# Kateridge/TransMF_AD

Hardware: AMD Instinct MI355X
Metric: volume-pairs/sec fwd+bwd(+Adam), 96^3 MRI+PET batch=8 per GPU (higher is better)
Workload: dtype f32

## Files before the change

### transmf_ad_amd/csrc/conv1_fused.hip

```cpp
#include <type_traits>
#include "conv1_z.h"

namespace {
using namespace c1z;

enum { MODE_STATS = 0, MODE_FWD = 1, MODE_REDUCE = 2, MODE_WGRAD = 3, MODE_RD = 4 };
#ifndef TMF_C1X_LAZY
#define TMF_C1X_LAZY 0x12
#endif

struct Args {
    const float* x;
    const float* w;
    const float* scale;
    const float* shift;
    const float* mean;
    const float* invstd;
    const float* coef;
    const void* dpool;
    void* pooled;
    float* zsel;
    unsigned char* parg;
    float* partial;
    float* partial2;
    int D, H, W, C;
    int tilesD, tilesH, tilesW, ntiles, tiles_per_block;
    float slope;
};

template <int MODE, bool BF16, bool P16 = false, bool SPLIT = false, bool ROUTE = false>
__global__ __launch_bounds__(256, (MODE == 3 && !SPLIT) || (MODE == 1 && SPLIT) ? 4 : 2) void conv1_fused_kernel(Args a) {
    static_assert(!(BF16 && SPLIT), "SPLIT is the fp32 mode's variant");
    static_assert(!ROUTE || (!BF16 && !P16 && (MODE == MODE_FWD || (MODE == MODE_RD && !SPLIT))),
                  "ROUTE: the fp32 forward (either form of z) and the one-pass backward, which evaluates no z and so has one form");
    constexpr bool NOZ = ROUTE && MODE == MODE_RD;
    constexpr bool B16L = BF16 || SPLIT;
    constexpr int NIMG = SPLIT ? 3 : 1;
    constexpr bool KEEP32 = SPLIT && (MODE == MODE_RD || MODE == MODE_WGRAD);
    __shared__ float halo[B16L ? NIMG * NHB_DW : NHALO];
    __shared__ float halo32[KEEP32 ? NHALO : 1];
    const unsigned hb_base = (unsigned)(size_t)(__attribute__((address_space(3))) const void*)halo;
    __shared__ float red[4 * 32 * 32];
    const int tid = threadIdx.x;
    const int lane = tid & 63;
    const int wave = __builtin_amdgcn_readfirstlane(tid >> 6);
    const int l31 = lane & 31, hsel = lane >> 5;
    const int n0 = blockIdx.y * 32;
    const int co = n0 + l31;
    const bool cv = co < a.C;
    const int OD = a.D / 2, OH = a.H / 2, OW = a.W / 2;

    float bw[B16L ? 1 : 14];
    tmf_bf16x8 bwb[NIMG][3];
    if constexpr (B16L) weights_b16<SPLIT>(a.w, a.C, co, cv, hsel, bwb);
    else if constexpr (!NOZ) weights_f32(a.w, a.C, co, cv, hsel, bw);
    float sc = 0.f, sh = 0.f, mu = 0.f, is = 0.f, c0 = 0.f, c1 = 0.f;
    if (MODE != MODE_STATS && cv) { sc = a.scale[co]; sh = a.shift[co]; }
    if ((MODE == MODE_REDUCE || MODE == MODE_WGRAD || MODE == MODE_RD) && cv) { mu = a.mean[co]; is = a.invstd[co]; }
    if (MODE == MODE_WGRAD && cv) { c0 = a.coef[co]; c1 = a.coef[a.C + co]; }

    float s1 = 0.f, s2 = 0.f;
    float dacc[MODE == MODE_RD ? 27 : 1];
#pragma unroll
    for (int t = 0; t < (MODE == MODE_RD ? 27 : 1); ++t) dacc[t] = 0.f;
    f32x16 accw;
#pragma unroll
    for (int r = 0; r < 16; ++r) accw[r] = 0.f;
    const int a_tap = tapoff(l31);
    const int wg_tap = l31 < 27 ? l31 : 0, wg_c = (wg_tap % 3) & 1;
    const unsigned wg_b = hb_base + 2u * (unsigned)((wg_tap / 9) * BPLANE + ((wg_tap / 3) % 3) * BROW + wg_tap % 3 + wg_c +
                                                    wg_c * BCOPY + 2 * hsel * BROW);

    const int tile_begin = blockIdx.x * a.tiles_per_block;
    int tile_end = tile_begin + a.tiles_per_block;
    if (tile_end > a.ntiles) tile_end = a.ntiles;

    constexpr int OOB = (int)0x80000000u;
    constexpr int HVN = (NHALO + 255) / 256;
    float hv[HVN];
    int hrel[HVN], hcrd[HVN], hdst[HVN];
#pragma unroll
    for (int q = 0; q < HVN; ++q) {
        const int e = tid + q * 256;
        const int hw = e % HW, hh = (e / HW) % HH, hd = e / (HW * HH);
        hrel[q] = e < NHALO ? ((hd * a.H + hh) * a.W + hw) * 4 : OOB;
        hcrd[q] = hd | hh << 8 | hw << 16;
        hdst[q] = hd * BPLANE + hh * BROW + hw;
    }
    if (B16L) {
        for (int e = tid; e < NIMG * NHB_DW; e += 256) halo[e] = 0.f;
        __syncthreads();
    }
    auto min_i = [](int x_, int y_) { return x_ < y_ ? x_ : y_; };
    struct Crd { int tw, th, td, b; long xoff; bool in_dh, full_dh; };
    const bool even_dims = (a.D % 2 == 0) && (a.H % 2 == 0) && (a.W % 2 == 0);
    auto row_setup = [&](Crd& c) {
        const int d0 = c.td * TD, h0 = c.th * TH;
        c.xoff = (long)c.b * a.D * a.H * a.W + ((long)((d0 - 1) * a.H + (h0 - 1)) * a.W + (c.tw * TW - 1));
        c.in_dh = d0 >= 1 && d0 + TD < a.D && h0 >= 1 && h0 + TH < a.H;
        c.full_dh = d0 + TD <= a.D && h0 + TH <= a.H && even_dims;
    };
    auto next_crd = [&](Crd c) {
        c.xoff += TW;
        if (++c.tw == a.tilesW) {
            c.tw = 0;
            if (++c.th == a.tilesH) {
                c.th = 0;
                if (++c.td == a.tilesD) { c.td = 0; ++c.b; }
            }
            row_setup(c);
        }
        return c;
    };
    auto fetch = [&](const Crd& c) {
        const int d0 = c.td * TD, h0 = c.th * TH, w0 = c.tw * TW;
        const float* org = a.x + c.xoff;
        const __amdgpu_buffer_rsrc_t xr = __builtin_amdgcn_make_buffer_rsrc(const_cast<float*>(org), 0, 0x7FFFFFFF, 0x00020000);
        if (c.in_dh && w0 >= 1 && w0 + TW < a.W) {
#pragma unroll
            for (int q = 0; q < HVN; ++q)
                hv[q] = __builtin_bit_cast(float, __builtin_amdgcn_raw_buffer_load_b32(xr, hrel[q], 0, 0));
        } else {
            const int lo = (d0 == 0 ? 1 : 0) | (h0 == 0 ? 1 : 0) << 8 | (w0 == 0 ? 1 : 0) << 16;
            const int hi = min_i(HD - 1, a.D - d0) | min_i(HH - 1, a.H - h0) << 8 | min_i(HW - 1, a.W - w0) << 16;
            const unsigned lo_bias = 0x808080u - (unsigned)lo, hi_bias = (unsigned)hi | 0x808080u;
#pragma unroll
            for (int q = 0; q < HVN; ++q) {
                const unsigned tt = (unsigned)hcrd[q] + lo_bias, uu = hi_bias - (unsigned)hcrd[q];
                const int off = (((tt & uu) | ~0x808080u) == 0xFFFFFFFFu) ? hrel[q] : OOB;
                hv[q] = __builtin_bit_cast(float, __builtin_amdgcn_raw_buffer_load_b32(xr, off, 0, 0));
            }
        }
    };
    constexpr int PSZ = P16 ? 2 : 4;
    const int pl_lane = cv ? (hsel * OW * a.C + co) * PSZ : OOB;
    Crd cur;
    {
        int t = tile_begin;
        cur.tw = t % a.tilesW; t /= a.tilesW;
        cur.th = t % a.tilesH; t /= a.tilesH;
        cur.td = t % a.tilesD;
        cur.b = t / a.tilesD;
        row_setup(cur);
    }
    if (tile_begin < tile_end) fetch(cur);
    for (int tile = tile_begin; tile < tile_end; ++tile) {
        const int b = cur.b;
        const int d0 = cur.td * TD, h0 = cur.th * TH, w0 = cur.tw * TW;
        const bool full = cur.full_dh && w0 + TW <= a.W;
        cur = next_crd(cur);
        if (tile > tile_begin) __syncthreads();
        constexpr bool REDST = SPLIT && ROUTE && MODE == MODE_FWD;
        int tid_b = tid;
        if (REDST) asm volatile("" : "+v"(tid_b));
#pragma unroll
        for (int q = 0; q < HVN; ++q) {
            const int e = tid + q * 256;
            if (REDST) {
                const int eb = tid_b + q * 256;
                hdst[q] = (eb / (HW * HH)) * BPLANE + ((eb / HW) % HH) * BROW + eb % HW;
            }
            if (SPLIT) {
                if (e < NHALO) {
                    store_halo_split(halo, hdst[q], hv[q]);
                    if (KEEP32) halo32[e] = hv[q];
                }
            } else if (BF16) {
                if (e < NHALO) store_halo_bf16(halo, hdst[q], hv[q]);
            } else {
                if (e < NHALO) halo[e] = hv[q];
            }
        }
        __syncthreads();
        if (tile + 1 < tile_end) fetch(cur);

        auto process = [&](auto full_c) {
        constexpr bool FULL = decltype(full_c)::value;
        f32x16 zt[NTI];
        constexpr bool LAZY = (BF16 && MODE == MODE_WGRAD) || (SPLIT && ((TMF_C1X_LAZY >> MODE) & 1));
        const int i = l31;
        const unsigned lane_b = lane_base(hb_base, i, hsel);
        auto conv_tiles = [&](f32x16* zp, int mt0, auto n_c) {
            constexpr int N = decltype(n_c)::value;
            if constexpr (B16L) conv_tiles_b16<SPLIT, N>(zp, lane_b, mt0, bwb);
            else conv_tiles_f32<N>(zp, halo, mt0, vox_off(i), hsel, bw);
        };
        if (!LAZY && !NOZ) conv_tiles(zt, wave * NTI, std::integral_constant<int, NTI>{});
#pragma unroll
        for (int ti = 0; ti < NTI; ++ti) {
            const int mt = wave * NTI + ti;
            const int org = tile_org(mt);
            if (LAZY) conv_tiles(&zt[ti], mt, std::integral_constant<int, 1>{});
            f32x16& z = zt[ti];
            const int bd = d0 + 2 * (mt >> 2), bh = h0 + 4 * ((mt >> 1) & 1) + 2 * hsel, bwid = w0 + 4 * (mt & 1);

            if (MODE == MODE_STATS) {
#pragma unroll
                for (int r = 0; r < 16; ++r) {
                    const int gd = bd + ((r >> 2) & 1), gh = bh + ((r >> 1) & 1), gw = bwid + 2 * ((r >> 3) & 1) + (r & 1);
                    if (FULL || (gd < a.D && gh < a.H && gw < a.W)) { s1 += z[r]; s2 += z[r] * z[r]; }
                }
                continue;
            }

            float K0 = 0.f, K1 = 0.f;
            if (MODE == MODE_WGRAD) {
                K1 = -sc * c1 * is;
                K0 = sc * (c1 * mu * is - c0);
            }
            const int od = (d0 >> 1) + (mt >> 2), ohb = (h0 >> 1) + 2 * ((mt >> 1) & 1), owb = (w0 >> 1) + 2 * (mt & 1);
            void* pbase = MODE == MODE_FWD ? a.pooled : const_cast<void*>(a.dpool);
            const __amdgpu_buffer_rsrc_t pr = __builtin_amdgcn_make_buffer_rsrc(
                reinterpret_cast<char*>(pbase) + (size_t)b * OD * OH * OW * a.C * PSZ, 0, OD * OH * OW * a.C * PSZ, 0x00020000);
            const int pv = (FULL || ohb + hsel < OH) ? pl_lane : OOB;
            const __amdgpu_buffer_rsrc_t zr = __builtin_amdgcn_make_buffer_rsrc(
                reinterpret_cast<char*>(a.zsel) + (ROUTE ? (size_t)b * OD * OH * OW * a.C * 4 : 0), 0, ROUTE ? OD * OH * OW * a.C * 4 : 0, 0x00020000);
            const __amdgpu_buffer_rsrc_t ar = __builtin_amdgcn_make_buffer_rsrc(
                a.parg + (ROUTE ? (size_t)b * OD * OH * OW * a.C : 0), 0, ROUTE ? OD * OH * OW * a.C : 0, 0x00020000);
#pragma unroll
            for (int q = 0; q < 2; ++q) {
                const int ow = owb + q;
                const bool win_u = FULL || (od < OD && ow < OW);
                const int psoff = ((od * OH + ohb) * OW + ow) * a.C * PSZ;
                if (NOZ) {
                    float g = 0.f, zs = 0.f;
                    int arg = 0;
                    if (win_u) {
                        g = __builtin_bit_cast(float, __builtin_amdgcn_raw_buffer_load_b32(pr, pv, psoff, 0));
                        zs = __builtin_bit_cast(float, __builtin_amdgcn_raw_buffer_load_b32(zr, pv, psoff, 0));
                        arg = __builtin_amdgcn_raw_buffer_load_b8(ar, (int)((unsigned)pv >> 2), psoff / PSZ, 0) & 7;
                    }
                    const float gl = g * (zs * sc + sh > 0.f ? 1.f : a.slope);
                    s1 += gl;
                    s2 += gl * ((zs - mu) * is);
                    const int vx = org + hsel * 2 * HW + ((arg >> 2) & 1) * HH * HW + ((arg >> 1) & 1) * HW + 2 * q + (arg & 1);
#pragma unroll
                    for (int t = 0; t < 27; ++t) dacc[t] = fmaf(halo[vx + tapoff(t)], gl, dacc[t]);
                    continue;
                }
                float y[8];
                window_y(z, q, sc, sh, y);
                const float ymax = window_max(y);
                const float lrm = ymax > 0.f ? 1.f : a.slope;
                if (MODE == MODE_FWD) {
                    const float best = ymax * lrm;
                    if ((TMF_C1X_ABL & 1) && best == 12345.678f) __builtin_amdgcn_raw_buffer_store_b32(__builtin_bit_cast(unsigned, best), pr, pv, psoff, 0);
                    if (win_u && !(TMF_C1X_ABL & 1)) {
                        if (P16) __builtin_amdgcn_raw_buffer_store_b16((unsigned short)(tmf_pack_bf16(best, 0.f) & 0xFFFFu), pr, pv, psoff, 0);
                        else __builtin_amdgcn_raw_buffer_store_b32(__builtin_bit_cast(unsigned, best), pr, pv, psoff, 0);
                        if (ROUTE) {
                            const float zs = window_zsel(y, ymax, z, q);
                            const int arg = window_arg(y, ymax);
                            __builtin_amdgcn_raw_buffer_store_b32(__builtin_bit_cast(unsigned, zs), zr, pv, psoff, 0);
                            __builtin_amdgcn_raw_buffer_store_b8((unsigned char)arg, ar, (int)((unsigned)pv >> 2), psoff / PSZ, 0);
                        }
                    }
                    continue;
                }
                float g = 0.f;
                if (win_u)
                    g = P16 ? __builtin_bit_cast(float, (unsigned int)__builtin_amdgcn_raw_buffer_load_b16(pr, pv, psoff, 0) << 16)
                            : __builtin_bit_cast(float, __builtin_amdgcn_raw_buffer_load_b32(pr, pv, psoff, 0));
                const float gl = g * lrm;
                if (MODE == MODE_REDUCE || MODE == MODE_RD) {
                    const float zs = window_zsel(y, ymax, z, q);
                    s1 += gl;
                    s2 += gl * ((zs - mu) * is);
                    if (MODE == MODE_RD) {
                        const int arg = window_arg(y, ymax);
                        if (BF16) {
                            const int hd = 2 * (mt >> 2) + ((arg >> 2) & 1), hh = 4 * ((mt >> 1) & 1) + 2 * hsel + ((arg >> 1) & 1);
                            const unsigned short* hb = reinterpret_cast<const unsigned short*>(halo) + hd * BPLANE + hh * BROW +
                                                       4 * (mt & 1) + 2 * q + (arg & 1);
#pragma unroll
                            for (int t = 0; t < 27; ++t) {
                                const float xv = __builtin_bit_cast(float, (unsigned int)hb[(t / 9) * BPLANE + ((t / 3) % 3) * BROW + t % 3] << 16);
                                dacc[t] = fmaf(xv, gl, dacc[t]);
                            }
                        } else {
                        const int vx = org + hsel * 2 * HW + ((arg >> 2) & 1) * HH * HW + ((arg >> 1) & 1) * HW + 2 * q + (arg & 1);
                        const float* h32 = KEEP32 ? halo32 : halo;
#pragma unroll
                        for (int t = 0; t < 27; ++t) dacc[t] = fmaf(h32[vx + tapoff(t)], gl, dacc[t]);
                        }
                    }
                } else {
                    const int arg = window_arg(y, ymax);
                    const float add = sc * gl;
#pragma unroll
                    for (int k = 0; k < 8; ++k) {
                        const int r = 8 * q + k;
                        const int gd = bd + ((r >> 2) & 1), gh = bh + ((r >> 1) & 1), gw = bwid + 2 * q + (r & 1);
                        const bool vv = FULL || (gd < a.D && gh < a.H && gw < a.W);
                        const float dzv = z[r] * K1 + K0 + (k == arg ? add : 0.f);
                        z[r] = (vv && cv) ? dzv : 0.f;
                    }
                }
            }
            if (MODE == MODE_WGRAD) {
                const int a_row = org + hsel * 2 * HW + a_tap;
                if (BF16) {
                    const unsigned wt = wg_b + 2u * (unsigned)((2 * (mt >> 2)) * BPLANE + 4 * ((mt >> 1) & 1) * BROW + 4 * (mt & 1));
#pragma unroll
                    for (int m = 0; m < 2; ++m) {
                        float bv[8];
                        unsigned ad[4];
#pragma unroll
                        for (int u = 0; u < 4; ++u)
                            ad[u] = *reinterpret_cast<const __attribute__((address_space(3))) unsigned*>(
                                (size_t)(wt + 2u * (unsigned)((u >> 1) * BPLANE + (u & 1) * BROW + 2 * m)));
#pragma unroll
                        for (int j = 0; j < 8; ++j) bv[j] = z[8 * m + j];
                        const tmf_u32x4 av = {ad[0], ad[1], ad[2], ad[3]};
                        accw = __builtin_amdgcn_mfma_f32_32x32x16_bf16(__builtin_bit_cast(tmf_bf16x8, av), pack8(bv), accw, 0, 0, 0);
                    }
                } else {
#pragma unroll
                    for (int r = 0; r < 16; ++r)
                        accw = __builtin_amdgcn_mfma_f32_32x32x2f32((KEEP32 ? halo32 : halo)[a_row + row_off(r)], z[r], accw, 0, 0, 0);
                }
            }
        }
        };
        if (full)
            process(std::true_type{});
        else
            process(std::false_type{});
    }

    if (MODE == MODE_STATS || MODE == MODE_REDUCE || MODE == MODE_RD) {
        s1 += __shfl_xor(s1, 32);
        s2 += __shfl_xor(s2, 32);
        __syncthreads();
        if (hsel == 0) { red[(wave * 32 + l31) * 2] = s1; red[(wave * 32 + l31) * 2 + 1] = s2; }
        __syncthreads();
        if (tid < 32 && n0 + tid < a.C) {
            float t1 = 0.f, t2 = 0.f;
#pragma unroll
            for (int m = 0; m < 4; ++m) { t1 += red[(m * 32 + tid) * 2]; t2 += red[(m * 32 + tid) * 2 + 1]; }
            a.partial[((size_t)blockIdx.x * 2 + 0) * a.C + n0 + tid] = t1;
            a.partial[((size_t)blockIdx.x * 2 + 1) * a.C + n0 + tid] = t2;
        }
    }
    if (MODE == MODE_RD) {
        __syncthreads();
#pragma unroll
        for (int t = 0; t < 27; ++t) {
            const float v = dacc[t] + __shfl_xor(dacc[t], 32);
            if (hsel == 0) red[(wave * 32 + t) * 32 + l31] = v;
        }
        __syncthreads();
        for (int e = tid; e < 27 * 32; e += 256) {
            const int tap = e >> 5, c = e & 31;
            if (n0 + c < a.C) {
                const float v = red[(0 * 32 + tap) * 32 + c] + red[(1 * 32 + tap) * 32 + c] +
                                red[(2 * 32 + tap) * 32 + c] + red[(3 * 32 + tap) * 32 + c];
                a.partial2[((size_t)blockIdx.x * 27 + tap) * a.C + n0 + c] = v;
            }
        }
    } else if (MODE == MODE_WGRAD) {
        __syncthreads();
#pragma unroll
        for (int r = 0; r < 16; ++r) {
            const int tap = (r & 3) + 8 * (r >> 2) + 4 * hsel;
            red[(wave * 32 + tap) * 32 + l31] = accw[r];
        }
        __syncthreads();
        for (int e = tid; e < 27 * 32; e += 256) {
            const int tap = e >> 5, c = e & 31;
            if (n0 + c < a.C) {
                const float v = red[(0 * 32 + tap) * 32 + c] + red[(1 * 32 + tap) * 32 + c] +
                                red[(2 * 32 + tap) * 32 + c] + red[(3 * 32 + tap) * 32 + c];
                a.partial[((size_t)blockIdx.x * 27 + tap) * a.C + n0 + c] = v;
            }
        }
    }
}

struct Plan { int tilesD, tilesH, tilesW, ntiles, nby, tpb, nblk; };
Plan make_plan(int B, int D, int H, int W, int C, int target_blocks) {
    Plan p;
    p.tilesD = tmf_cdiv(D, TD); p.tilesH = tmf_cdiv(H, TH); p.tilesW = tmf_cdiv(W, TW);
    p.ntiles = B * p.tilesD * p.tilesH * p.tilesW;
    p.nby = tmf_cdiv(C, 32);
    int want = target_blocks / p.nby;
    if (want < 1) want = 1;
    if (want > p.ntiles) want = p.ntiles;
    p.tpb = tmf_cdiv(p.ntiles, want);
    p.nblk = tmf_cdiv(p.ntiles, p.tpb);
    return p;
}
#define SLAB_BLOCKS tmf_opt(TMF_OPT_C1_BLOCKS)

int check(const char* fn, int B, int D, int H, int W, int C) { return check_shape(fn, B, D, H, W, C); }

Args base_args(const float* x, const float* w, int D, int H, int W, int C, const Plan& p, float slope) {
    Args a = {};
    a.x = x; a.w = w; a.D = D; a.H = H; a.W = W; a.C = C;
    a.tilesD = p.tilesD; a.tilesH = p.tilesH; a.tilesW = p.tilesW; a.ntiles = p.ntiles; a.tiles_per_block = p.tpb;
    a.slope = slope;
    return a;
}

int c1_split_mode() { return tmf_opt(TMF_OPT_C1_SPLIT); }

}

extern "C" int tmf_c1_blocks(int B, int D, int H, int W, int C) {
    if (B <= 0 || D <= 0 || H <= 0 || W <= 0 || C <= 0) return 0;
    return make_plan(B, D, H, W, C, SLAB_BLOCKS).nblk;
}

static int c1_stats(bool bf16, const float* x, const float* w, float* stat_partial,
                    int B, int D, int H, int W, int C, void* stream) {
    TMF_REQUIRE_PTR(x); TMF_REQUIRE_PTR(w); TMF_REQUIRE_PTR(stat_partial);
    int rc = check("tmf_c1_stats", B, D, H, W, C);
    if (rc) return rc;
    const Plan p = make_plan(B, D, H, W, C, SLAB_BLOCKS);
    Args a = base_args(x, w, D, H, W, C, p, 0.f);
    a.partial = stat_partial;
    if (bf16) hipLaunchKernelGGL((conv1_fused_kernel<MODE_STATS, true>), dim3(p.nblk, p.nby), dim3(256), 0, (hipStream_t)stream, a);
    else if (c1_split_mode()) hipLaunchKernelGGL((conv1_fused_kernel<MODE_STATS, false, false, true>), dim3(p.nblk, p.nby), dim3(256), 0, (hipStream_t)stream, a);
    else      hipLaunchKernelGGL((conv1_fused_kernel<MODE_STATS, false>), dim3(p.nblk, p.nby), dim3(256), 0, (hipStream_t)stream, a);
    return tmf_launch_result("tmf_c1_stats");
}
extern "C" int tmf_c1_stats(const float* x, const float* w, float* stat_partial,
                            int B, int D, int H, int W, int C, void* stream) {
    return c1_stats(false, x, w, stat_partial, B, D, H, W, C, stream);
}
extern "C" int tmf_c1_stats_bf16(const float* x, const float* w, float* stat_partial,
                                 int B, int D, int H, int W, int C, void* stream) {
    return c1_stats(true, x, w, stat_partial, B, D, H, W, C, stream);
}

static int c1_bn_pool_fwd(bool bf16, bool p16, const float* x, const float* w, const float* scale, const float* shift,
                          void* pooled, int B, int D, int H, int W, int C, float slope, void* stream,
                          float* z_sel = nullptr, unsigned char* arg = nullptr) {
    TMF_REQUIRE_PTR(x); TMF_REQUIRE_PTR(w); TMF_REQUIRE_PTR(scale); TMF_REQUIRE_PTR(shift); TMF_REQUIRE_PTR(pooled);
    int rc = check("tmf_c1_bn_pool_fwd", B, D, H, W, C);
    if (rc) return rc;
    const Plan p = make_plan(B, D, H, W, C, tmf_opt(TMF_OPT_C1_FWD_MULT) * SLAB_BLOCKS);
    Args a = base_args(x, w, D, H, W, C, p, slope);
    a.scale = scale; a.shift = shift; a.pooled = pooled; a.zsel = z_sel; a.parg = arg;
    TMF_REQUIRE(bf16 || !p16, TMF_E_ARG, "tmf_c1_bn_pool_fwd: bf16 tensors only with the bf16 kernels");
    if (z_sel != nullptr) {
        if (c1_split_mode()) hipLaunchKernelGGL((conv1_fused_kernel<MODE_FWD, false, false, true, true>), dim3(p.nblk, p.nby), dim3(256), 0, (hipStream_t)stream, a);
        else                 hipLaunchKernelGGL((conv1_fused_kernel<MODE_FWD, false, false, false, true>), dim3(p.nblk, p.nby), dim3(256), 0, (hipStream_t)stream, a);
        return tmf_launch_result("tmf_c1_bn_pool_fwd_route");
    }
    if (bf16 && p16) hipLaunchKernelGGL((conv1_fused_kernel<MODE_FWD, true, true>), dim3(p.nblk, p.nby), dim3(256), 0, (hipStream_t)stream, a);
    else if (bf16)   hipLaunchKernelGGL((conv1_fused_kernel<MODE_FWD, true>), dim3(p.nblk, p.nby), dim3(256), 0, (hipStream_t)stream, a);
    else if (c1_split_mode()) hipLaunchKernelGGL((conv1_fused_kernel<MODE_FWD, false, false, true>), dim3(p.nblk, p.nby), dim3(256), 0, (hipStream_t)stream, a);
    else             hipLaunchKernelGGL((conv1_fused_kernel<MODE_FWD, false>), dim3(p.nblk, p.nby), dim3(256), 0, (hipStream_t)stream, a);
    return tmf_launch_result("tmf_c1_bn_pool_fwd");
}
extern "C" int tmf_c1_bn_pool_fwd(const float* x, const float* w, const float* scale, const float* shift,
                                  float* pooled, int B, int D, int H, int W, int C, float slope, void* stream) {
    return c1_bn_pool_fwd(false, false, x, w, scale, shift, pooled, B, D, H, W, C, slope, stream);
}
extern "C" int tmf_c1_bn_pool_fwd_route(const float* x, const float* w, const float* scale, const float* shift, float* pooled,
                                        float* z_sel, unsigned char* arg, int B, int D, int H, int W, int C, float slope, void* stream) {
    TMF_REQUIRE_PTR(z_sel); TMF_REQUIRE_PTR(arg);
    return c1_bn_pool_fwd(false, false, x, w, scale, shift, pooled, B, D, H, W, C, slope, stream, z_sel, arg);
}
extern "C" int tmf_c1_bn_pool_fwd_bf16(const float* x, const float* w, const float* scale, const float* shift,
                                       void* pooled, int B, int D, int H, int W, int C, float slope, int pooled_bf16,
                                       void* stream) {
    return c1_bn_pool_fwd(true, pooled_bf16 != 0, x, w, scale, shift, pooled, B, D, H, W, C, slope, stream);
}

static int c1_bwd_reduce(bool bf16, bool p16, const float* x, const float* w, const float* scale, const float* shift,
                         const float* mean, const float* invstd, const void* dpool, float* partial,
                         int B, int D, int H, int W, int C, float slope, void* stream) {
    TMF_REQUIRE_PTR(x); TMF_REQUIRE_PTR(w); TMF_REQUIRE_PTR(scale); TMF_REQUIRE_PTR(shift);
    TMF_REQUIRE_PTR(mean); TMF_REQUIRE_PTR(invstd); TMF_REQUIRE_PTR(dpool); TMF_REQUIRE_PTR(partial);
    int rc = check("tmf_c1_bwd_reduce", B, D, H, W, C);
    if (rc) return rc;
    const Plan p = make_plan(B, D, H, W, C, SLAB_BLOCKS);
    Args a = base_args(x, w, D, H, W, C, p, slope);
    a.scale = scale; a.shift = shift; a.mean = mean; a.invstd = invstd; a.dpool = dpool; a.partial = partial;
// ... 144 lines not shown
```

### transmf_ad_amd/csrc/conv3d_mfma.hip

```cpp
#include <type_traits>
#include "tmf_device.h"

#ifndef TMF_CONV_ACC
#define TMF_CONV_ACC 1
#endif
#ifndef TMF_CONV_BUF
#define TMF_CONV_BUF 1
#endif

namespace {

template <int KS_, int CINC_, int MT_, int NT_, int WM_, int WN_, int TD_, int TH_, int TW_, int TPS_>
struct FwdCfg {
    static constexpr int KS = KS_, CINC = CINC_, MT = MT_, NT = NT_, WM = WM_, WN = WN_;
    static constexpr int TD = TD_, TH = TH_, TW = TW_, TPS = TPS_;
    static constexpr int PAD = KS / 2;
    static constexpr int HD = TD + 2 * PAD, HH = TH + 2 * PAD, HW = TW + 2 * PAD;
    static constexpr int NHALO = HD * HH * HW;
    static constexpr int CP = CINC + 4;
    static constexpr int NPOS = TD * TH * TW;
    static constexpr int NB = 32 * NT * WN;
    static constexpr int NTAPS = KS * KS * KS;
    static constexpr int NSTAGES = NTAPS / TPS;
    static constexpr int BSTAGE = TPS * CINC * NB;
// ... 997 lines not shown
                    } else {
#pragma unroll
                        for (int u = 0; u < 4; ++u)
                            if (c + u < Cin) v[u] = src[u];
                    }
                }
                hreg[q] = v;
            }
        }
    };
    auto fetch_dz = [&](int tile) {
        int b, d0, h0, w0;
        locate(tile, b, d0, h0, w0);
        const float* dzb = dz + (size_t)b * D * H * W * Cout;
        if constexpr (BUF) {
            const float* org = dzb + ((long)(d0 * H + h0) * W + w0) * Cout;
            const __amdgpu_buffer_rsrc_t dr = __builtin_amdgcn_make_buffer_rsrc(const_cast<float*>(org), 0, 0x7FFFFFFF, 0x00020000);
            if (d0 + C::TD <= D && h0 + C::TH <= H && w0 + C::TW <= W) {
#pragma unroll
                for (int q = 0; q < DV; ++q)
                    dreg[q] = __builtin_bit_cast(f32x4, __builtin_amdgcn_raw_buffer_load_b128(dr, drel[q], 0, 0));
            } else {
                const int hi = min_i(C::TD, D - d0) - 1 | (min_i(C::TH, H - h0) - 1) << 8 | (min_i(C::TW, W - w0) - 1) << 16;
                const int hi_bias = hi | 0x808080;
#pragma unroll
                for (int q = 0; q < DV; ++q) {
                    const int off = in_box(dcrd[q], 0x808080, hi_bias) ? drel[q] : OOB;
                    dreg[q] = __builtin_bit_cast(f32x4, __builtin_amdgcn_raw_buffer_load_b128(dr, off, 0, 0));
                }
            }
        } else {
#pragma unroll
            for (int q = 0; q < DV; ++q) {
                const int e = tid + q * C::NTHR;
                const int p = e / (C::NB / 4), c4 = e % (C::NB / 4);
                const int pw = p % C::TW, ph = (p / C::TW) % C::TH, pd = p / (C::TW * C::TH);
                const int gd = d0 + pd, gh = h0 + ph, gw = w0 + pw;
                const int c = co0 + c4 * 4;
                f32x4 v = {0.f, 0.f, 0.f, 0.f};
                if (e < C::NPOS * (C::NB / 4) && gd < D && gh < H && gw < W) {
                    const float* src = dzb + ((size_t)(gd * H + gh) * W + gw) * Cout + c;
                    if (VEC) {
                        if (c < Cout) v = *reinterpret_cast<const f32x4*>(src);
                    } else {
#pragma unroll
                        for (int u = 0; u < 4; ++u)
                            if (c + u < Cout) v[u] = src[u];
                    }
                }
                dreg[q] = v;
            }
        }
    };

    constexpr bool DZ_AHEAD = C::NT == 1;
    if (tile_begin < tile_end) {
        fetch_halo(tile_begin, 0, HVP);
        if (DZ_AHEAD) fetch_dz(tile_begin);
    }
    for (int tile = tile_begin; tile < tile_end; ++tile) {
        if ((dbg & 1) && tile > tile_begin) goto compute;
        fetch_halo(tile, HVP, HV);
        if (!DZ_AHEAD) fetch_dz(tile);
        __syncthreads();
#pragma unroll
        for (int q = 0; q < HV; ++q) {
            const int e = tid + q * C::NTHR;
            if (e < C::NHALO * C4) *reinterpret_cast<f32x4*>(&xh[e * 4]) = hreg[q];
        }
#pragma unroll
        for (int q = 0; q < DV; ++q) {
            const int e = tid + q * C::NTHR;
            if (e < C::NPOS * (C::NB / 4)) *reinterpret_cast<f32x4*>(&dzs[e * 4]) = dreg[q];
        }
        __syncthreads();
        if (tile + 1 < tile_end) {
            fetch_halo(tile + 1, 0, HVP);
            if (DZ_AHEAD) fetch_dz(tile + 1);
        }

    compute:
        if (dbg & 2) continue;
        auto mma_bricks = [&](auto ntaps_c) {
            constexpr int NTAPS = decltype(ntaps_c)::value;
#pragma unroll 1
            for (int pd = 0; pd < C::TD; ++pd) {
                const float* xp[NTAPS];
#pragma unroll
                for (int t = 0; t < NTAPS; ++t) xp[t] = xh + tapoff[t] + pd * C::HH * C::HW * C::CI;
                const float* bsrc = dzs + b_lane + pd * C::TH * C::TW * C::NB;
#pragma unroll
                for (int ph = 0; ph < C::TH; ++ph) {
#pragma unroll
                    for (int q = 0; q < C::TW / 2; ++q) {
                        float bv[C::NT], av[NTAPS];
#pragma unroll
                        for (int j = 0; j < C::NT; ++j) bv[j] = bsrc[(ph * C::TW + 2 * q) * C::NB + j * 32];
#pragma unroll
                        for (int t = 0; t < NTAPS; ++t) av[t] = xp[t][ph * C::HW * C::CI + 2 * q * C::CI];
#pragma unroll
                        for (int t = 0; t < NTAPS; ++t)
#pragma unroll
                            for (int j = 0; j < C::NT; ++j)
                                acc[t][j] = __builtin_amdgcn_mfma_f32_32x32x2f32(av[t], bv[j], acc[t][j], 0, 0, 0);
                    }
                }
            }
        };
        if (C::PACK) {
            if (wave < 6) mma_bricks(std::integral_constant<int, 2>{});
            else mma_bricks(std::integral_constant<int, 1>{});
        }
        else if (C::NW == 4) mma_bricks(std::integral_constant<int, C::TPW>{});
        else if (wave < 4) mma_bricks(std::integral_constant<int, 4>{});
        else mma_bricks(std::integral_constant<int, 3>{});
    }

#pragma unroll
    for (int t = 0; t < C::TPW; ++t) {
        const int tap0 = C::PACK ? 2 * (wave + 8 * t) : tap_base + t;
        if (t < tap_cnt && tap0 < 27) {
#pragma unroll
            for (int j = 0; j < C::NT; ++j) {
                const int co = co0 + j * 32 + l31;
#pragma unroll
                for (int r = 0; r < 16; ++r) {
                    const int m = (r & 3) + 8 * (r >> 2) + 4 * hsel;
                    const int tap = C::PACK ? tap0 + (r >> 3) : tap0;
                    const int ci = ci0 + (C::PACK ? (m & 15) : m);
                    if (tap < 27 && ci < Cin && co < Cout)
                        partial[(((size_t)split * 27 + tap) * Cin + ci) * Cout + co] = acc[t][j][r];
                }
            }
        }
    }
}

template <int NT>
__global__ __launch_bounds__(256) void conv1x1_wgrad_kernel(
    const float* __restrict__ x, const float* __restrict__ dz, float* __restrict__ partial,
    long npos, int Cin, int Cout, int slabs_per_block) {
    const int tid = threadIdx.x;
    const int lane = tid & 63;
    const int wave = __builtin_amdgcn_readfirstlane(tid >> 6);
    const int l31 = lane & 31, hsel = lane >> 5;
    const int ci = blockIdx.y * 32 + l31;
    const int co0 = blockIdx.z * 32 * NT;
    f32x16 acc[NT];
#pragma unroll
    for (int j = 0; j < NT; ++j)
#pragma unroll
        for (int r = 0; r < 16; ++r) acc[j][r] = 0.f;
    const long p_begin = ((long)blockIdx.x * slabs_per_block) * 256 + wave * 64;
    for (int sl = 0; sl < slabs_per_block; ++sl) {
        const long pb = p_begin + (long)sl * 256;
#pragma unroll 8
        for (int q = 0; q < 32; ++q) {
            const long p = pb + 2 * q + hsel;
            const bool pv = p < npos;
            const float av = (pv && ci < Cin) ? x[p * Cin + ci] : 0.f;
#pragma unroll
            for (int j = 0; j < NT; ++j) {
                const int co = co0 + j * 32 + l31;
                const float bv = (pv && co < Cout) ? dz[p * Cout + co] : 0.f;
                acc[j] = __builtin_amdgcn_mfma_f32_32x32x2f32(av, bv, acc[j], 0, 0, 0);
            }
        }
    }
    const int split = blockIdx.x * 4 + wave;
#pragma unroll
    for (int j = 0; j < NT; ++j) {
        const int co = co0 + j * 32 + l31;
#pragma unroll
        for (int r = 0; r < 16; ++r) {
            const int cr = blockIdx.y * 32 + (r & 3) + 8 * (r >> 2) + 4 * hsel;
            if (cr < Cin && co < Cout) partial[((size_t)split * Cin + cr) * Cout + co] = acc[j][r];
        }
    }
}

struct WgPlan {
    int nt, tilesD, tilesH, tilesW, ntiles, tps, nsplit, gy, gz;
    int small;
    int pack;
};

WgPlan plan_wgrad(int B, int D, int H, int W, int cin, int cout) {
    WgPlan p;
    const int mind = D < H ? (D < W ? D : W) : (H < W ? H : W);
    p.small = !(mind >= 16 || (long)D * H * W >= 4096);
    const int td = 4, th = p.small ? 4 : 8, tw = p.small ? 4 : 8;
    const bool w8 = (cin % 4 == 0) && (cout % 4 == 0) && conv_waves() >= 8;
    p.nt = (cout <= 32 || w8) ? 1 : 2;
    p.tilesD = tmf_cdiv(D, td); p.tilesH = tmf_cdiv(H, th); p.tilesW = tmf_cdiv(W, tw);
    p.ntiles = B * p.tilesD * p.tilesH * p.tilesW;
    p.pack = w8 && cin <= 16;
    p.gy = p.pack ? 1 : tmf_cdiv(cin, 32);
    p.gz = tmf_cdiv(cout, 32 * p.nt);
    const int groups = p.gy * p.gz;
    int want = 256 / groups;
    if (want < 1) want = 1;
    if (want > p.ntiles) want = p.ntiles;
    p.tps = tmf_cdiv(p.ntiles, want);
    p.nsplit = tmf_cdiv(p.ntiles, p.tps);
    return p;
}

struct Wg1Plan { int nt, gy, gz, spb, nblk, nsplit; };
Wg1Plan plan_wgrad1(long npos, int cin, int cout) {
    Wg1Plan p;
    p.nt = cout <= 32 ? 1 : 2;
    p.gy = tmf_cdiv(cin, 32);
    p.gz = tmf_cdiv(cout, 32 * p.nt);
    const long slabs = (npos + 255) / 256;
    int want = 1024 / (p.gy * p.gz);
    if (want < 1) want = 1;
    if (want > slabs) want = (int)slabs;
    p.spb = (int)((slabs + want - 1) / want);
    p.nblk = (int)((slabs + p.spb - 1) / p.spb);
    p.nsplit = p.nblk * 4;
    return p;
}

constexpr int C1_TD = 4, C1_TH = 8, C1_TW = 8;
constexpr int C1_HD = C1_TD + 2, C1_HH = C1_TH + 2, C1_HW = C1_TW + 2;
constexpr int C1_NHALO = C1_HD * C1_HH * C1_HW;

__device__ __forceinline__ constexpr int c1_tapoff(int tap) {
    return tap >= 27 ? 0 : ((tap / 9) * C1_HH + (tap / 3) % 3) * C1_HW + tap % 3;
}

__global__ __launch_bounds__(256) void conv3d_c1_fwd_kernel(
    const float* __restrict__ x, const float* __restrict__ w, float* __restrict__ z,
    float* __restrict__ stat_partial, int D, int H, int W, int Cout,
    int tilesD, int tilesH, int tilesW, int ntiles) {
    __shared__ float halo[C1_NHALO];
    __shared__ float red[4 * 32 * 2];
    const int tid = threadIdx.x;
    const int lane = tid & 63;
    const int wave = __builtin_amdgcn_readfirstlane(tid >> 6);
    const int l31 = lane & 31, hsel = lane >> 5;
    const int tile = xcd_contiguous(blockIdx.x, ntiles);
    int t = tile;
    const int tw = t % tilesW; t /= tilesW;
    const int th = t % tilesH; t /= tilesH;
    const int td = t % tilesD;
    const int b = t / tilesD;
    const int d0 = td * C1_TD, h0 = th * C1_TH, w0 = tw * C1_TW;
    const int n0 = blockIdx.y * 32;
    const int co = n0 + l31;

    const float* xb = x + (size_t)b * D * H * W;
    for (int e = tid; e < C1_NHALO; e += 256) {
        const int hw = e % C1_HW, hh = (e / C1_HW) % C1_HH, hd = e / (C1_HW * C1_HH);
        const int gd = d0 + hd - 1, gh = h0 + hh - 1, gw = w0 + hw - 1;
        float v = 0.f;
        if (gd >= 0 && gd < D && gh >= 0 && gh < H && gw >= 0 && gw < W)
            v = xb[(size_t)(gd * H + gh) * W + gw];
        halo[e] = v;
    }
    float bw[14];
#pragma unroll
    for (int s = 0; s < 14; ++s) {
        const int tap = 2 * s + hsel;
        bw[s] = (tap < 27 && co < Cout) ? w[tap * Cout + co] : 0.f;
    }
    __syncthreads();

    f32x16 acc[2];
    int abase[2];
#pragma unroll
    for (int i = 0; i < 2; ++i) {
#pragma unroll
        for (int r = 0; r < 16; ++r) acc[i][r] = 0.f;
        const int p = (wave * 2 + i) * 32 + l31;
        const int pw = p % C1_TW, ph = (p / C1_TW) % C1_TH, pd = p / (C1_TW * C1_TH);
        abase[i] = (pd * C1_HH + ph) * C1_HW + pw;
    }
#pragma unroll
    for (int s = 0; s < 14; ++s) {
        const int off = hsel ? c1_tapoff(2 * s + 1) : c1_tapoff(2 * s);
#pragma unroll
        for (int i = 0; i < 2; ++i)
            acc[i] = __builtin_amdgcn_mfma_f32_32x32x2f32(halo[abase[i] + off], bw[s], acc[i], 0, 0, 0);
    }

    float s1 = 0.f, s2 = 0.f;
    float* zb = z + (size_t)b * D * H * W * Cout;
#pragma unroll
    for (int i = 0; i < 2; ++i) {
#pragma unroll
        for (int r = 0; r < 16; ++r) {
            const int p = (wave * 2 + i) * 32 + (r & 3) + 8 * (r >> 2) + 4 * hsel;
            const int pw = p % C1_TW, ph = (p / C1_TW) % C1_TH, pd = p / (C1_TW * C1_TH);
            const int gd = d0 + pd, gh = h0 + ph, gw = w0 + pw;
            if (gd < D && gh < H && gw < W && co < Cout) {
                const float v = acc[i][r];
                zb[((size_t)(gd * H + gh) * W + gw) * Cout + co] = v;
                s1 += v;
                s2 += v * v;
            }
        }
    }
    if (stat_partial != nullptr) {
        s1 += __shfl_xor(s1, 32);
        s2 += __shfl_xor(s2, 32);
        if (hsel == 0) {
            red[(wave * 32 + l31) * 2 + 0] = s1;
            red[(wave * 32 + l31) * 2 + 1] = s2;
        }
        __syncthreads();
        if (tid < 32 && n0 + tid < Cout) {
            float a1 = 0.f, a2 = 0.f;
#pragma unroll
            for (int m = 0; m < 4; ++m) {
                a1 += red[(m * 32 + tid) * 2 + 0];
                a2 += red[(m * 32 + tid) * 2 + 1];
            }
            stat_partial[((size_t)tile * 2 + 0) * Cout + n0 + tid] = a1;
            stat_partial[((size_t)tile * 2 + 1) * Cout + n0 + tid] = a2;
// ... 283 lines not shown
```

Before: 1037.

## Prefetch pooled gradients one tile ahead and double-buffer 1x1 wgrad loads

In the one-pass routed backward conv1 kernel, the pooled gradient, selected z and argmax for the next tile are now loaded into a ping-pong register set alongside the halo prefetch. Previously they were loaded inside the compute loop. The kernel is also retuned to 3 waves per SIMD occupancy and always takes the full-tile path. Separately, the 1x1 weight-gradient kernel now issues buffer loads in double-buffered pieces ahead of the MFMAs, replacing the old per-iteration guarded global loads. The goal is to hide memory latency behind compute, at the cost of more registers and some scheduling barriers.

```diff
diff --git a/transmf_ad_amd/csrc/conv1_fused.hip b/transmf_ad_amd/csrc/conv1_fused.hip
--- a/transmf_ad_amd/csrc/conv1_fused.hip
+++ b/transmf_ad_amd/csrc/conv1_fused.hip
@@ -29,7 +29,7 @@
 };
 
 template <int MODE, bool BF16, bool P16 = false, bool SPLIT = false, bool ROUTE = false>
-__global__ __launch_bounds__(256, (MODE == 3 && !SPLIT) || (MODE == 1 && SPLIT) ? 4 : 2) void conv1_fused_kernel(Args a) {
+__global__ __launch_bounds__(256, (MODE == 3 && !SPLIT) || (MODE == 1 && SPLIT) ? 4 : (ROUTE && MODE == 4) ? 3 : 2) void conv1_fused_kernel(Args a) {
     static_assert(!(BF16 && SPLIT), "SPLIT is the fp32 mode's variant");
     static_assert(!ROUTE || (!BF16 && !P16 && (MODE == MODE_FWD || (MODE == MODE_RD && !SPLIT))),
                   "ROUTE: the fp32 forward (either form of z) and the one-pass backward, which evaluates no z and so has one form");
@@ -112,10 +112,10 @@
         }
         return c;
     };
-    auto fetch = [&](const Crd& c) {
+    auto fetch = [&](const Crd& c, bool live = true) {
         const int d0 = c.td * TD, h0 = c.th * TH, w0 = c.tw * TW;
         const float* org = a.x + c.xoff;
-        const __amdgpu_buffer_rsrc_t xr = __builtin_amdgcn_make_buffer_rsrc(const_cast<float*>(org), 0, 0x7FFFFFFF, 0x00020000);
+        const __amdgpu_buffer_rsrc_t xr = __builtin_amdgcn_make_buffer_rsrc(const_cast<float*>(org), 0, live ? 0x7FFFFFFF : 0, 0x00020000);
         if (c.in_dh && w0 >= 1 && w0 + TW < a.W) {
 #pragma unroll
             for (int q = 0; q < HVN; ++q)
@@ -143,8 +143,39 @@
         cur.b = t / a.tilesD;
         row_setup(cur);
     }
-    if (tile_begin < tile_end) fetch(cur);
-    for (int tile = tile_begin; tile < tile_end; ++tile) {
+    struct Pool { float g[NTI][2], zs[NTI][2]; unsigned char arg[NTI][2]; };
+    Pool pool_a, pool_b;
+    auto fetch_pool = [&](const Crd& c, Pool& s, bool live) {
+        const int d0 = c.td * TD, h0 = c.th * TH, w0 = c.tw * TW;
+        const bool full = c.full_dh && w0 + TW <= a.W;
+        const int nwc = live ? OD * OH * OW * a.C : 0;
+        const __amdgpu_buffer_rsrc_t pr = __builtin_amdgcn_make_buffer_rsrc(
+            reinterpret_cast<char*>(const_cast<void*>(a.dpool)) + (size_t)c.b * nwc * 4, 0, nwc * 4, 0x00020000);
+        const __amdgpu_buffer_rsrc_t zr = __builtin_amdgcn_make_buffer_rsrc(
+            reinterpret_cast<char*>(a.zsel) + (size_t)c.b * nwc * 4, 0, nwc * 4, 0x00020000);
+        const __amdgpu_buffer_rsrc_t ar = __builtin_amdgcn_make_buffer_rsrc(a.parg + (size_t)c.b * nwc, 0, nwc, 0x00020000);
+#pragma unroll
+        for (int ti = 0; ti < NTI; ++ti) {
+            const int mt = wave * NTI + ti;
+            const int od = (d0 >> 1) + (mt >> 2), ohb = (h0 >> 1) + 2 * ((mt >> 1) & 1), owb = (w0 >> 1) + 2 * (mt & 1);
+            const int pv = (full || ohb + hsel < OH) ? pl_lane : OOB;
+#pragma unroll
+            for (int q = 0; q < 2; ++q) {
+                const int ow = owb + q;
+                const bool win_u = full || (od < OD && ow < OW);
+                const int psoff = win_u ? ((od * OH + ohb) * OW + ow) * a.C * 4 : 0;
+                const int po = win_u ? pv : OOB;
+                s.g[ti][q] = __builtin_bit_cast(float, __builtin_amdgcn_raw_buffer_load_b32(pr, po, psoff, 0));
+                s.zs[ti][q] = __builtin_bit_cast(float, __builtin_amdgcn_raw_buffer_load_b32(zr, po, psoff, 0));
+                s.arg[ti][q] = __builtin_amdgcn_raw_buffer_load_b8(ar, (int)((unsigned)po >> 2), psoff / 4, 0);
+            }
+        }
+    };
+    if (tile_begin < tile_end) {
+        fetch(cur);
+        if constexpr (NOZ) fetch_pool(cur, pool_a, true);
+    }
+    auto brick = [&](const int tile, const Pool& pc, Pool& pn) __attribute__((always_inline)) {
         const int b = cur.b;
         const int d0 = cur.td * TD, h0 = cur.th * TH, w0 = cur.tw * TW;
         const bool full = cur.full_dh && w0 + TW <= a.W;
@@ -172,7 +203,14 @@
             }
         }
         __syncthreads();
-        if (tile + 1 < tile_end) fetch(cur);
+        if constexpr (NOZ) {
+            const bool live = tile + 1 < tile_end;
+            fetch(cur, live);
+            fetch_pool(cur, pn, live);
+            __builtin_amdgcn_sched_barrier(0);
+        } else if (tile + 1 < tile_end) {
+            fetch(cur);
+        }
 
         auto process = [&](auto full_c) {
         constexpr bool FULL = decltype(full_c)::value;
@@ -223,19 +261,19 @@
                 const bool win_u = FULL || (od < OD && ow < OW);
                 const int psoff = ((od * OH + ohb) * OW + ow) * a.C * PSZ;
                 if (NOZ) {
-                    float g = 0.f, zs = 0.f;
-                    int arg = 0;
-                    if (win_u) {
-                        g = __builtin_bit_cast(float, __builtin_amdgcn_raw_buffer_load_b32(pr, pv, psoff, 0));
-                        zs = __builtin_bit_cast(float, __builtin_amdgcn_raw_buffer_load_b32(zr, pv, psoff, 0));
-                        arg = __builtin_amdgcn_raw_buffer_load_b8(ar, (int)((unsigned)pv >> 2), psoff / PSZ, 0) & 7;
-                    }
+                    const float g = pc.g[ti][q], zs = pc.zs[ti][q];
+                    const int arg = pc.arg[ti][q] & 7;
                     const float gl = g * (zs * sc + sh > 0.f ? 1.f : a.slope);
                     s1 += gl;
                     s2 += gl * ((zs - mu) * is);
                     const int vx = org + hsel * 2 * HW + ((arg >> 2) & 1) * HH * HW + ((arg >> 1) & 1) * HW + 2 * q + (arg & 1);
 #pragma unroll
                     for (int t = 0; t < 27; ++t) dacc[t] = fmaf(halo[vx + tapoff(t)], gl, dacc[t]);
+#pragma unroll
+                    for (int t = 0; t < 27; t += 9)
+                        asm volatile("" : "+v"(dacc[t]), "+v"(dacc[t + 1]), "+v"(dacc[t + 2]), "+v"(dacc[t + 3]), "+v"(dacc[t + 4]),
+                                          "+v"(dacc[t + 5]), "+v"(dacc[t + 6]), "+v"(dacc[t + 7]), "+v"(dacc[t + 8]));
+                    __builtin_amdgcn_sched_barrier(0);
                     continue;
                 }
                 float y[8];
@@ -322,10 +360,18 @@
             }
         }
         };
-        if (full)
+        if (NOZ || full)
             process(std::true_type{});
         else
             process(std::false_type{});
+    };
+    if constexpr (NOZ) {
+        for (int tile = tile_begin; tile < tile_end; tile += 2) {
+            brick(tile, pool_a, pool_b);
+            if (tile + 1 < tile_end) brick(tile + 1, pool_b, pool_a);
+        }
+    } else {
+        for (int tile = tile_begin; tile < tile_end; ++tile) brick(tile, pool_a, pool_a);
     }
 
     if (MODE == MODE_STATS || MODE == MODE_REDUCE || MODE == MODE_RD) {
diff --git a/transmf_ad_amd/csrc/conv3d_mfma.hip b/transmf_ad_amd/csrc/conv3d_mfma.hip
--- a/transmf_ad_amd/csrc/conv3d_mfma.hip
+++ b/transmf_ad_amd/csrc/conv3d_mfma.hip
@@ -1173,20 +1173,56 @@
 #pragma unroll
         for (int r = 0; r < 16; ++r) acc[j][r] = 0.f;
     const long p_begin = ((long)blockIdx.x * slabs_per_block) * 256 + wave * 64;
+    constexpr int OOB = (int)0x80000000u;
+    constexpr int HQ = 8, NPH = 32 / HQ;
+    const int x_lane = ci < Cin ? (hsel * Cin + ci) * 4 : OOB;
+    int d_lane[NT];
+#pragma unroll
+    for (int j = 0; j < NT; ++j) {
+        const int co = co0 + j * 32 + l31;
+        d_lane[j] = co < Cout ? (hsel * Cout + co) * 4 : OOB;
+    }
+    float xa[2][HQ], da[2][HQ][NT];
+    auto request = [&](int sl, auto piece_c) {
+        constexpr int PIECE = decltype(piece_c)::value, SET = PIECE & 1;
+        const long pb = p_begin + (long)sl * 256 + PIECE * 2 * HQ;
+        long left = sl < slabs_per_block ? npos - pb : 0;
+        left = left < 0 ? 0 : (left > 2 * HQ ? 2 * HQ : left);
+        const long pc = left > 0 ? pb : 0;
+        const __amdgpu_buffer_rsrc_t xr = __builtin_amdgcn_make_buffer_rsrc(const_cast<float*>(x + pc * Cin), 0, (int)left * Cin * 4, 0x00020000);
+        const __amdgpu_buffer_rsrc_t dr = __builtin_amdgcn_make_buffer_rsrc(const_cast<float*>(dz + pc * Cout), 0, (int)left * Cout * 4, 0x00020000);
+#pragma unroll
+        for (int q = 0; q < HQ; ++q) {
+            xa[SET][q] = __builtin_bit_cast(float, __builtin_amdgcn_raw_buffer_load_b32(xr, x_lane, 2 * q * Cin * 4, 0));
+#pragma unroll
+            for (int j = 0; j < NT; ++j)
+                da[SET][q][j] = __builtin_bit_cast(float, __builtin_amdgcn_raw_buffer_load_b32(dr, d_lane[j], 2 * q * Cout * 4, 0));
+        }
+        __builtin_amdgcn_sched_barrier(0);
+    };
+    auto multiply = [&](auto set_c) {
+        constexpr int SET = decltype(set_c)::value;
+#pragma unroll
+        for (int q = 0; q < HQ; ++q)
+#pragma unroll
+            for (int j = 0; j < NT; ++j)
+                acc[j] = __builtin_amdgcn_mfma_f32_32x32x2f32(xa[SET][q], da[SET][q][j], acc[j], 0, 0, 0);
+        __builtin_amdgcn_sched_barrier(0);
+    };
+    auto phase = [&](int sl, auto ph_c) {
+        constexpr int PH = decltype(ph_c)::value;
+        multiply(std::integral_constant<int, PH & 1>{});
+        if constexpr (PH + 2 < NPH) request(sl, std::integral_constant<int, PH + 2>{});
+        else request(sl + 1, std::integral_constant<int, PH + 2 - NPH>{});
+    };
+    request(0, std::integral_constant<int, 0>{});
+    request(0, std::integral_constant<int, 1>{});
+#pragma unroll 1
     for (int sl = 0; sl < slabs_per_block; ++sl) {
-        const long pb = p_begin + (long)sl * 256;
-#pragma unroll 8
-        for (int q = 0; q < 32; ++q) {
-            const long p = pb + 2 * q + hsel;
-            const bool pv = p < npos;
-            const float av = (pv && ci < Cin) ? x[p * Cin + ci] : 0.f;
-#pragma unroll
-            for (int j = 0; j < NT; ++j) {
-                const int co = co0 + j * 32 + l31;
-                const float bv = (pv && co < Cout) ? dz[p * Cout + co] : 0.f;
-                acc[j] = __builtin_amdgcn_mfma_f32_32x32x2f32(av, bv, acc[j], 0, 0, 0);
-            }
-        }
+        phase(sl, std::integral_constant<int, 0>{});
+        phase(sl, std::integral_constant<int, 1>{});
+        phase(sl, std::integral_constant<int, 2>{});
+        phase(sl, std::integral_constant<int, 3>{});
     }
     const int split = blockIdx.x * 4 + wave;
 #pragma unroll
```

Result: no change. 1043, median of 6 (+0.7%).
